# williamyang1991/FRESCO

Measured on AMD Instinct MI355X. Metric: denoising-steps/sec (8-frame batch, 512^2), FRESCO hot-path step, higher is better.
Workload: dtype f16; 1 GPU; cfg2 (BASELINE.json configs[1]): 8 frames 512x512, SD-1.5 decoder shapes, FRESCO attention only (3x up_blocks.2 HW=1024 C=640 + 3x up_blocks.3 HW=4096 C=320 processor calls per step, projections included), 15-step schedule 1x spatial+cf+temporal / 7x cf+temporal / 7x cf; parallelism=single GPU

## Files before the change

### fresco_amd/csrc/attn.hip

```cpp
#include "attn_cfg.h"
#include <type_traits>

namespace fresco {

template <int D>
__global__ __launch_bounds__(256) void kv_pack_kernel(const half_t* __restrict__ k,
                                                       const half_t* __restrict__ v,
                                                       const int32_t* __restrict__ kv_rows,
                                                       char* __restrict__ img, float* __restrict__ ktmax,
                                                       int H, int M, int nT, int64_t group_rows,
                                                       int64_t kv_ld) {
    using Cfg = AttnCfg<D>;
    const int tile = blockIdx.x, h = blockIdx.y, g = blockIdx.z;
    __shared__ int32_t rows[64];
    __shared__ __attribute__((aligned(16))) half_t ks[64][D + 8];
    __shared__ __attribute__((aligned(16))) half_t vs[64][D + 8];

    if (threadIdx.x < 64) {
        const int m = tile * 64 + threadIdx.x;
        int32_t r = -1;
        if (m < M) r = kv_rows ? kv_rows[m] : m;
        rows[threadIdx.x] = r;
    }
    __syncthreads();
// ... 30 lines not shown
        for (int e = 0; e < 8; ++e) {
            const int key = kc * 16 + (e & 3) + 8 * (e >> 2) + 4 * cc;
            half_t val = (half_t)0;
            if (d < D)
                val = vs[key][d];
            else if (Cfg::ONES && d == D && rows[key] >= 0)
                val = (half_t)1;
            o[e] = val;
        }
        *reinterpret_cast<half8_t*>(dst + Cfg::TILE + Cfg::KTILE + (int64_t)c * 16) = o;
    }
    {
        const int row = threadIdx.x >> 2, part = threadIdx.x & 3;
        float n2 = 0.f;
        for (int dc = part; dc < D / 8; dc += 4) {
            const half8_t kk = *reinterpret_cast<const half8_t*>(&ks[row][dc * 8]);
#pragma unroll
            for (int e = 0; e < 8; ++e) n2 = fmaf((float)kk[e], (float)kk[e], n2);
        }
        n2 += __shfl_xor(n2, 1, 64);
        n2 += __shfl_xor(n2, 2, 64);
#pragma unroll
        for (int off = 32; off >= 4; off >>= 1) n2 = fmaxf(n2, __shfl_xor(n2, off, 64));
        __shared__ float wmax[4];
        if ((threadIdx.x & 63) == 0) wmax[threadIdx.x >> 6] = n2;
        __syncthreads();
        if (threadIdx.x == 0)
            ktmax[(int64_t)(g * H + h) * nT + tile] = fmaxf(fmaxf(wmax[0], wmax[1]), fmaxf(wmax[2], wmax[3]));
    }
}

template <int KIN, int D>
struct KvProjCfg {
    static constexpr int ROWB = KIN * 2 + 16;
    static constexpr int HPW = 160 / D;
    static constexpr int NPART = D / 4;
    static constexpr int XS_BYTES = 64 * ROWB;
    static constexpr int LDS_BYTES = XS_BYTES + HPW * NPART * 64 * 4 + 64 * 4;
};

template <int KIN, int D>
__global__ __launch_bounds__(320, KIN == 320 ? 3 : 2) void kvproj_pack_kernel(const half_t* __restrict__ x, int64_t x_ld,
                                                           const int32_t* __restrict__ x_rows,
                                                           const half_t* __restrict__ Wk,
                                                           const half_t* __restrict__ Wv, char* __restrict__ img,
                                                           float* __restrict__ ktmax, int H, int M, int nT) {
    using Cfg = AttnCfg<D>;
    using PC = KvProjCfg<KIN, D>;
    constexpr int ROWB = PC::ROWB, HPW = PC::HPW, NPART = PC::NPART;
    constexpr int NKS = KIN / 16;
    constexpr int SK = 4;
    constexpr int NST = NKS / SK;
    constexpr int CPR = KIN / 8;
    constexpr int NXL = 64 * CPR / 320;
    static_assert(NKS % SK == 0 && (64 * CPR) % 320 == 0 && 160 % D == 0 && D % 8 == 0, "shapes");
    extern __shared__ __attribute__((aligned(16))) char smem[];
    char* xs = smem;
    float* n2p = reinterpret_cast<float*>(smem + PC::XS_BYTES);
    int32_t* rows = reinterpret_cast<int32_t*>(n2p + HPW * NPART * 64);
    const int tile = blockIdx.x, fg = blockIdx.y, g = blockIdx.z;
    const int tid = threadIdx.x, lane = tid & 63, wave = tid >> 6;
    const int l31 = lane & 31, hi = lane >> 5;

    if (tid < 64) {
        const int m = tile * 64 + tid;
        rows[tid] = m < M ? x_rows[(int64_t)g * M + m] : -1;
    }
    const int ft = fg * 5 + wave;
    const half_t* wkp = Wk + (int64_t)(ft * 32 + l31) * KIN + hi * 32;
    const half_t* wvp = Wv + (int64_t)(ft * 32 + l31) * KIN + hi * 32;
    half8_t fk[2][SK], fv[2][SK];
    auto fetch = [&](int st, int buf) __attribute__((always_inline)) {
#pragma unroll
        for (int i = 0; i < SK; ++i) {
            fk[buf][i] = *reinterpret_cast<const half8_t*>(wkp + st * 64 + i * 8);
            fv[buf][i] = *reinterpret_cast<const half8_t*>(wvp + st * 64 + i * 8);
        }
    };
    fetch(0, 0);
    __builtin_amdgcn_sched_barrier(0);
    __syncthreads();
    {
        uint4 xv[NXL];
#pragma unroll
        for (int i = 0; i < NXL; ++i) {
            const int c = tid + i * 320;
            const int row = c / CPR, dc = c % CPR;
            const int32_t r = rows[row];
            xv[i] = make_uint4(0, 0, 0, 0);
            if (r >= 0) xv[i] = *reinterpret_cast<const uint4*>(x + (int64_t)r * x_ld + dc * 8);
        }
        __builtin_amdgcn_sched_barrier(0);
#pragma unroll
        for (int i = 0; i < NXL; ++i) {
            const int c = tid + i * 320;
            *reinterpret_cast<uint4*>(xs + (c / CPR) * ROWB + (c % CPR) * 16) = xv[i];
        }
    }
    floatx16 ak[2], av[2];
#pragma unroll
    for (int b = 0; b < 2; ++b)
#pragma unroll
        for (int r = 0; r < 16; ++r) ak[b][r] = av[b][r] = 0.f;
    __syncthreads();
#pragma unroll
    for (int st = 0; st < NST; ++st) {
        const int buf = st & 1;
        if (st + 1 < NST) fetch(st + 1, buf ^ 1);
        __builtin_amdgcn_sched_barrier(0);
#pragma unroll
        for (int i = 0; i < SK; ++i) {
            const int kb = (st * 64 + hi * 32 + i * 8) * 2;
            const half8_t x0 = *reinterpret_cast<const half8_t*>(xs + l31 * ROWB + kb);
            const half8_t x1 = *reinterpret_cast<const half8_t*>(xs + (32 + l31) * ROWB + kb);
            ak[0] = __builtin_amdgcn_mfma_f32_32x32x16_f16(fk[buf][i], x0, ak[0], 0, 0, 0);
            ak[1] = __builtin_amdgcn_mfma_f32_32x32x16_f16(fk[buf][i], x1, ak[1], 0, 0, 0);
            av[0] = __builtin_amdgcn_mfma_f32_32x32x16_f16(x0, fv[buf][i], av[0], 0, 0, 0);
            av[1] = __builtin_amdgcn_mfma_f32_32x32x16_f16(x1, fv[buf][i], av[1], 0, 0, 0);
        }
        __builtin_amdgcn_sched_barrier(0);
    }
#pragma unroll
    for (int b = 0; b < 2; ++b) {
        const int key = b * 32 + l31;
#pragma unroll
        for (int j = 0; j < 4; ++j) {
            const int f0 = ft * 32 + 8 * j + 4 * hi;
            const int head = f0 / D, dd = f0 - head * D;
            half4_t w;
            float n2 = 0.f;
#pragma unroll
            for (int e = 0; e < 4; ++e) {
                w[e] = (half_t)ak[b][4 * j + e];
                n2 = fmaf((float)w[e], (float)w[e], n2);
            }
            char* dst = img + ((int64_t)(g * H + head) * (nT + 1) + tile) * Cfg::TILE;
            *reinterpret_cast<half4_t*>(dst + ((dd >> 3) * 64 + key) * 16 + (dd & 7) * 2) = w;
            n2p[((head - fg * HPW) * NPART + (dd >> 2)) * 64 + key] = n2;
        }
    }
    {
        const int f = ft * 32 + l31;
        const int head = f / D, d = f - head * D;
        char* dst = img + ((int64_t)(g * H + head) * (nT + 1) + tile + 1) * Cfg::TILE + Cfg::KTILE;
#pragma unroll
        for (int b = 0; b < 2; ++b)
#pragma unroll
            for (int kq = 0; kq < 2; ++kq) {
                half8_t w;
#pragma unroll
                for (int e = 0; e < 8; ++e) w[e] = (half_t)av[b][8 * kq + e];
                *reinterpret_cast<half8_t*>(dst + (((2 * b + kq) * 2 + hi) * Cfg::DPV + d) * 16) = w;
            }
    }
    {
        constexpr int KPAD = (Cfg::DPK - D) / 8;
        constexpr int VPAD = Cfg::DPV - D;
        constexpr int PER_HEAD = KPAD * 64 + VPAD * 8;
        for (int i = tid; i < HPW * PER_HEAD; i += 320) {
            const int hl = i / PER_HEAD, c = i % PER_HEAD;
            const int head = fg * HPW + hl;
            char* base = img + ((int64_t)(g * H + head) * (nT + 1) + tile) * Cfg::TILE;
            if (c < KPAD * 64) {
                const int pc = c / 64, key = c % 64;
                uint4 val = make_uint4(0, 0, 0, 0);
                if (Cfg::MCOL && pc == 0 && rows[key] >= 0) val.x = 0x3C00u;
                *reinterpret_cast<uint4*>(base + ((D / 8 + pc) * 64 + key) * 16) = val;
            } else {
                const int c2 = c - KPAD * 64;
                const int pr = c2 / 8, kcc = c2 % 8;
                const int kc = kcc >> 1, cc = kcc & 1;
                half8_t o;
#pragma unroll
                for (int e = 0; e < 8; ++e) {
                    const int key = kc * 16 + (e & 3) + 8 * (e >> 2) + 4 * cc;
                    o[e] = (Cfg::ONES && pr == 0 && rows[key] >= 0) ? (half_t)1 : (half_t)0;
                }
                *reinterpret_cast<half8_t*>(base + Cfg::TILE + Cfg::KTILE + (kcc * Cfg::DPV + D + pr) * 16) = o;
            }
        }
    }
    __syncthreads();
    if (wave < HPW) {
        float n2 = 0.f;
#pragma unroll
        for (int p_ = 0; p_ < NPART; ++p_) n2 += n2p[(wave * NPART + p_) * 64 + lane];
#pragma unroll
        for (int off = 32; off > 0; off >>= 1) n2 = fmaxf(n2, __shfl_xor(n2, off, 64));
        if (lane == 0) ktmax[(int64_t)(g * H + fg * HPW + wave) * nT + tile] = n2;
    }
}

template <int N>
__device__ __forceinline__ void ring_wait_barrier() {
    asm volatile("s_waitcnt vmcnt(%0) lgkmcnt(0)\n\ts_barrier" ::"n"(N) : "memory");
}

template <int D, int QB>
__global__ __launch_bounds__(512, 2) void attn_flash_kernel(const half_t* __restrict__ q,
                                                          const char* __restrict__ img,
                                                          const float* __restrict__ ktmax,
                                                          half_t* __restrict__ out, int B, int H, int Lq,
                                                          int M, int nT, int batch_per_group,
                                                          float scale_log2, float diag_bias_log2, int64_t q_ld) {
    using Cfg = AttnCfg<D>;
    extern __shared__ __attribute__((aligned(16))) char smem[];
    constexpr int ROWS = 256 * QB;

    const int nQblk = (Lq + ROWS - 1) / ROWS;
    const unsigned blk = blockIdx.x;
    const int h = blk % H;
    const int qblk = (blk / H) % nQblk;
    const int b = blk / (H * nQblk);
    const int g = b / batch_per_group;
    const int C = H * D;

    const int tid = threadIdx.x;
    const int lane = tid & 63, wave = tid >> 6;
    const int l31 = lane & 31, hi = lane >> 5;
    const int qrow0 = qblk * ROWS + wave * 32 * QB + l31;
    const int wave_s = __builtin_amdgcn_readfirstlane(wave);
    const int grpB = wave_s >= 4 ? 1 : 0;

    half8_t qf[QB][Cfg::NKS];
    float q2[QB];
#pragma unroll
    for (int j = 0; j < QB; ++j) {
        const int qr = qrow0 + 32 * j;
        const half_t* qp = q + ((int64_t)b * Lq + (qr < Lq ? qr : Lq - 1)) * q_ld + h * D;
        q2[j] = 0.f;
#pragma unroll
        for (int ks = 0; ks < Cfg::NKS; ++ks) {
            const int d0 = ks * 16 + hi * 8;
            half8_t t = {0, 0, 0, 0, 0, 0, 0, 0};
            if (d0 < D) t = *reinterpret_cast<const half8_t*>(qp + d0);
#pragma unroll
            for (int e = 0; e < 8; ++e) q2[j] = fmaf((float)t[e], (float)t[e], q2[j]);
            qf[j][ks] = t;
        }
        q2[j] += __shfl_xor(q2[j], 32, 64);
    }

    float kmax;
    {
        const float* km = ktmax + (int64_t)(g * H + h) * nT;
        float k2 = 0.f;
        for (int i = lane; i < nT; i += 64) k2 = fmaxf(k2, km[i]);
#pragma unroll
        for (int off = 32; off > 0; off >>= 1) k2 = fmaxf(k2, __shfl_xor(k2, off, 64));
        kmax = sqrtf(k2);
// ... 226 lines not shown
            for (int db = 0; db < Cfg::NDB; ++db)
#pragma unroll
                for (int j = 0; j < QB; ++j) {
                    o[j][db] = __builtin_amdgcn_mfma_f32_32x32x16_f16(vf[kc][db], pf[j][kc], o[j][db], 0, 0, 0);
                }
        __builtin_amdgcn_sched_barrier(0);
        if (!LAST) qk(kf);
        __builtin_amdgcn_s_setprio(0);
        __builtin_amdgcn_sched_barrier(0);
    };

    const std::integral_constant<bool, true> yes;
    const std::integral_constant<bool, false> no_last, no;
    const std::integral_constant<bool, true> fast;
    {
        int u = 0;
        if (nT > 1) {
            step(0, no_last, no);
            u = 1;
            if (!need_diag) {
                bool safe = true;
#pragma unroll
                for (int j = 0; j < QB; ++j) safe = safe && (cmul * (qbound[j] - m_run[j]) <= NOMAX_THR);
                nomax = __builtin_amdgcn_readfirstlane((int)__all(safe));
            }
            if (!need_diag)
                for (; u + 3 < nT; ++u) step(u, no_last, fast);
            for (; u < nT - 1; ++u) step(u, no_last, no);
        }
        nomax = 0;
        step(u, yes, no);
    }

#pragma unroll
    for (int j = 0; j < QB; ++j) {
        float l_tot;
        if (Cfg::ONES) {
            constexpr int rr = D % 32;
            l_tot = __shfl(o[j][D / 32][(rr & 3) + 4 * (rr >> 3)], l31 + 32 * ((rr >> 2) & 1), 64);
        } else {
            l_tot = l_run[j] + __shfl_xor(l_run[j], 32, 64);
        }
        const float inv = 1.f / l_tot;
        const int qr = qrow0 + 32 * j;
        {
            half_t* op = out + ((int64_t)b * Lq + (qr < Lq ? qr : 0)) * C + h * D;
#pragma unroll
            for (int db = 0; db < Cfg::NDB; ++db)
#pragma unroll
                for (int gp = 0; gp < 2; ++gp) {
                    const int dA = db * 32 + gp * 16;
                    if (dA >= D) continue;
                    half4_t wa, wb;
#pragma unroll
                    for (int jj = 0; jj < 4; ++jj) {
                        wa[jj] = (half_t)(o[j][db][(2 * gp) * 4 + jj] * inv);
                        wb[jj] = (half_t)(o[j][db][(2 * gp + 1) * 4 + jj] * inv);
                    }
                    if (dA + 8 < D) {
                        const u32x2 a = __builtin_bit_cast(u32x2, wa), bb = __builtin_bit_cast(u32x2, wb);
                        const auto s0 = __builtin_amdgcn_permlane32_swap(a[0], bb[0], false, false);
                        const auto s1 = __builtin_amdgcn_permlane32_swap(a[1], bb[1], false, false);
                        u32x4 st;
                        st[0] = s0[0]; st[1] = s1[0]; st[2] = s0[1]; st[3] = s1[1];
                        if (qr < Lq) *reinterpret_cast<u32x4*>(op + dA + hi * 8) = st;
                    } else if (qr < Lq) {
                        *reinterpret_cast<half4_t*>(op + dA + hi * 4) = wa;
                    }
                }
        }
    }
}

template <int D, int QB>
static int launch_flash(const half_t* q, const char* img, half_t* out, int B, int H, int Lq, int M, int nT,
                        int n_groups, float scale, float diag_bias, int64_t q_ld, const float* ktmax,
                        hipStream_t st) {
    using Cfg = AttnCfg<D>;
    if (int rc = allow_dyn_lds(&attn_flash_kernel<D, QB>, Cfg::LDS_BYTES)) return rc;
    const int nQblk = (Lq + 256 * QB - 1) / (256 * QB);
    const float log2e = 1.4426950408889634f;
    ProfScope ps(FRESCO_PROF_ATTN_FLASH, B * H, Lq, M, D, st);
    const int grid = H * nQblk * B;
    hipLaunchKernelGGL((attn_flash_kernel<D, QB>), dim3(grid), dim3(512), Cfg::LDS_BYTES, st, q, img,
                       ktmax, out, B, H, Lq, M, nT, B / n_groups, scale * log2e, diag_bias * log2e, q_ld);
    return check_launch();
}

template <int D>
static int launch_attn(const half_t* q, const half_t* k, const half_t* v, const int32_t* kv_rows,
                       half_t* out, char* ws, int B, int H, int Lq, int n_groups, int M,
                       int64_t group_rows, float scale, float diag_bias, int64_t q_ld, int64_t kv_ld,
                       hipStream_t st) {
    using Cfg = AttnCfg<D>;
    const int nT = ntiles_of(M);
    char* img = ws;
    float* ktmax = reinterpret_cast<float*>(ws + align_up((size_t)n_groups * H * (nT + 1) * Cfg::TILE, 256));
    dim3 pg(nT, H, n_groups);
    {
        ProfScope ps(FRESCO_PROF_KV_PACK, n_groups, H, M, D, st);
        hipLaunchKernelGGL((kv_pack_kernel<D>), pg, dim3(256), 0, st, k, v, kv_rows, img, ktmax, H, M, nT, group_rows,
                           kv_ld);
    }
    if constexpr (D <= 48 && Cfg::MCOL) {
        const int grid2 = H * ((Lq + 511) / 512) * B;
        if (Lq > 256 && grid2 < device_cus())
            return launch_flash<D, 1>(q, img, out, B, H, Lq, M, nT, n_groups, scale, diag_bias, q_ld, ktmax, st);
        return launch_flash<D, 2>(q, img, out, B, H, Lq, M, nT, n_groups, scale, diag_bias, q_ld, ktmax, st);
    } else {
        return launch_flash<D, 1>(q, img, out, B, H, Lq, M, nT, n_groups, scale, diag_bias, q_ld, ktmax, st);
    }
}

static size_t attn_ws_bytes(int n_groups, int H, int M, int D) {
    const size_t nT = ntiles_of(M);
    const size_t dpk = (D + 15) / 16 * 16, dpv = (D + 31) / 32 * 32;
    return align_up((size_t)n_groups * H * (nT + 1) * ((dpk + dpv) * 128), 256) +
           align_up((size_t)n_groups * H * nT * sizeof(float), 256);
}

}

using namespace fresco;

extern "C" size_t fresco_attn_workspace_bytes(int n_groups, int H, int M, int D) {
    if (n_groups <= 0 || H <= 0 || M <= 0 || D <= 0) return 0;
    return attn_ws_bytes(n_groups, H, M, D);
}

extern "C" int fresco_attn_fwd_ld(const void* q, const void* k, const void* v, const int32_t* kv_rows,
                                  void* out, void* workspace, size_t workspace_bytes, int B, int H,
                                  int Lq, int D, int n_groups, int M, int64_t group_rows, float scale,
                                  float diag_bias, int64_t q_ld, int64_t kv_ld, void* stream) {
    if (!q || !k || !v || !out || !workspace) return FRESCO_EINVAL;
    if (q_ld < (int64_t)H * D || kv_ld < (int64_t)H * D || q_ld % 8 != 0 || kv_ld % 8 != 0) return FRESCO_EINVAL;
    if (B <= 0 || H <= 0 || Lq <= 0 || D <= 0 || n_groups <= 0 || M <= 0 || group_rows <= 0)
        return FRESCO_EINVAL;
    if (B % n_groups != 0 || !(scale > 0.f)) return FRESCO_EINVAL;
    if (workspace_bytes < attn_ws_bytes(n_groups, H, M, D)) return FRESCO_EWORKSPACE;
    hipStream_t st = as_stream(stream);
    const half_t* qh = static_cast<const half_t*>(q);
    const half_t* kh = static_cast<const half_t*>(k);
    const half_t* vh = static_cast<const half_t*>(v);
    half_t* oh = static_cast<half_t*>(out);
    char* ws = static_cast<char*>(workspace);
#define FRESCO_ATTN_CASE(DD)                                                                       \
    case DD:                                                                                       \
        return launch_attn<DD>(qh, kh, vh, kv_rows, oh, ws, B, H, Lq, n_groups, M, group_rows, scale, \
                               diag_bias, q_ld, kv_ld, st);
    switch (D) {
        FRESCO_ATTN_CASE(8)
        FRESCO_ATTN_CASE(16)
        FRESCO_ATTN_CASE(32)
        FRESCO_ATTN_CASE(40)
        FRESCO_ATTN_CASE(64)
        FRESCO_ATTN_CASE(80)
        FRESCO_ATTN_CASE(96)
        FRESCO_ATTN_CASE(128)
        default:
            return FRESCO_EUNSUPPORTED;
    }
#undef FRESCO_ATTN_CASE
}

namespace fresco {
template <int KIN, int D>
static int launch_kvproj_attn(const half_t* q, const half_t* x, int64_t x_ld, const int32_t* x_rows, const half_t* Wk,
                              const half_t* Wv, half_t* out, char* ws, int B, int H, int Lq, int n_groups, int M,
                              float scale, int64_t q_ld, hipStream_t st) {
    using Cfg = AttnCfg<D>;
    const int nT = ntiles_of(M);
    char* img = ws;
    float* ktmax = reinterpret_cast<float*>(ws + align_up((size_t)n_groups * H * (nT + 1) * Cfg::TILE, 256));
    {
        ProfScope ps(FRESCO_PROF_KV_PACK, n_groups, H, M, -D, st);
        constexpr int lds = KvProjCfg<KIN, D>::LDS_BYTES;
        if (int rc = allow_dyn_lds(&kvproj_pack_kernel<KIN, D>, lds)) return rc;
        hipLaunchKernelGGL((kvproj_pack_kernel<KIN, D>), dim3(nT, H * D / 160, n_groups), dim3(320), lds, st, x, x_ld, x_rows,
                           Wk, Wv, img, ktmax, H, M, nT);
    }
    if constexpr (D <= 48 && Cfg::MCOL) {
        const int grid2 = H * ((Lq + 511) / 512) * B;
        if (Lq > 256 && grid2 < device_cus())
            return launch_flash<D, 1>(q, img, out, B, H, Lq, M, nT, n_groups, scale, 0.f, q_ld, ktmax, st);
        return launch_flash<D, 2>(q, img, out, B, H, Lq, M, nT, n_groups, scale, 0.f, q_ld, ktmax, st);
    } else {
        return launch_flash<D, 1>(q, img, out, B, H, Lq, M, nT, n_groups, scale, 0.f, q_ld, ktmax, st);
    }
}
}

extern "C" int fresco_attn_kvproj_supported(int H, int D, int K_in) {
    return (H > 0 && (int64_t)H * D == K_in && ((D == 40 && K_in == 320) || (D == 80 && K_in == 640))) ? 1 : 0;
}

extern "C" int fresco_attn_fwd_kvproj(const void* q, const void* x, int64_t x_ld, const int32_t* x_rows, const void* Wk,
                                      const void* Wv, void* out, void* workspace, size_t workspace_bytes, int B, int H,
                                      int Lq, int D, int n_groups, int M, int K_in, float scale, int64_t q_ld,
                                      void* stream) {
    if (!q || !x || !x_rows || !Wk || !Wv || !out || !workspace) return FRESCO_EINVAL;
    if (B <= 0 || H <= 0 || Lq <= 0 || D <= 0 || n_groups <= 0 || M <= 0 || K_in <= 0) return FRESCO_EINVAL;
    if (B % n_groups != 0 || !(scale > 0.f)) return FRESCO_EINVAL;
    if (q_ld < (int64_t)H * D || q_ld % 8 != 0 || x_ld < K_in || x_ld % 8 != 0) return FRESCO_EINVAL;
    if (!fresco_attn_kvproj_supported(H, D, K_in)) return FRESCO_EUNSUPPORTED;
    if (workspace_bytes < attn_ws_bytes(n_groups, H, M, D)) return FRESCO_EWORKSPACE;
    hipStream_t st = as_stream(stream);
    const half_t* qh = static_cast<const half_t*>(q);
    const half_t* xh = static_cast<const half_t*>(x);
    const half_t* wk = static_cast<const half_t*>(Wk);
    const half_t* wv = static_cast<const half_t*>(Wv);
    half_t* oh = static_cast<half_t*>(out);
    char* ws = static_cast<char*>(workspace);
    if (D == 40)
        return launch_kvproj_attn<320, 40>(qh, xh, x_ld, x_rows, wk, wv, oh, ws, B, H, Lq, n_groups, M, scale, q_ld, st);
    return launch_kvproj_attn<640, 80>(qh, xh, x_ld, x_rows, wk, wv, oh, ws, B, H, Lq, n_groups, M, scale, q_ld, st);
}

extern "C" int fresco_attn_fwd(const void* q, const void* k, const void* v, const int32_t* kv_rows,
                               void* out, void* workspace, size_t workspace_bytes, int B, int H,
                               int Lq, int D, int n_groups, int M, int64_t group_rows, float scale,
                               float diag_bias, void* stream) {
// ... 4 lines not shown
```

Measured before the change: 486.6 denoising-steps/sec.

## Stage KV-projection weights via LDS DMA ring and stage packed tiles in LDS

Rewrites the fused K/V projection-and-pack kernel so weights are streamed into a 3-slot swizzled LDS ring with global_load_lds DMA instead of per-lane register fetches. For the C=320 case each block now processes two 64-key tiles, which amortizes weight traffic. Output K/V tiles are assembled in LDS and written out with coalesced 16-byte copies, and key norms are recomputed from the staged tile. In exchange the kernel uses about 145KB of LDS, which likely caps occupancy at one block per CU despite the launch bounds, and it relies on inline asm with hand-managed waitcnt.

```diff
diff --git a/fresco_amd/csrc/attn.hip b/fresco_amd/csrc/attn.hip
--- a/fresco_amd/csrc/attn.hip
+++ b/fresco_amd/csrc/attn.hip
@@ -86,12 +86,27 @@
 
 template <int KIN, int D>
 struct KvProjCfg {
+    static constexpr int NKT = KIN == 320 ? 2 : 1;
+    static constexpr int NKEY = NKT * 64;
     static constexpr int ROWB = KIN * 2 + 16;
     static constexpr int HPW = 160 / D;
-    static constexpr int NPART = D / 4;
-    static constexpr int XS_BYTES = 64 * ROWB;
-    static constexpr int LDS_BYTES = XS_BYTES + HPW * NPART * 64 * 4 + 64 * 4;
+    static constexpr int KC = 64;
+    static constexpr int SLOT = 160 * KC * 2;
+    static constexpr int NSLOT = 3;
+    static constexpr int XS_BYTES = NKEY * ROWB;
+    static constexpr int RING_OFF = XS_BYTES;
+    static constexpr int ROWS_OFF = RING_OFF + NSLOT * SLOT;
+    static constexpr int LDS_BYTES = ROWS_OFF + NKEY * 4;
+    static constexpr int OUT_BYTES = HPW * NKT * AttnCfg<D>::TILE;
+    static_assert(OUT_BYTES <= ROWS_OFF && SLOT % (5 * 1024) == 0 && XS_BYTES % 16 == 0, "LDS plan");
 };
+
+static_assert(KvProjCfg<320, 40>::LDS_BYTES == 145920 && KvProjCfg<640, 80>::LDS_BYTES == 144640, "the header's LDS plan");
+
+template <int N>
+__device__ __forceinline__ void kvproj_wait_barrier() {
+    asm volatile("s_waitcnt vmcnt(%0) lgkmcnt(0)\n\ts_barrier" ::"n"(N) : "memory");
+}
 
 template <int KIN, int D>
 __global__ __launch_bounds__(320, KIN == 320 ? 3 : 2) void kvproj_pack_kernel(const half_t* __restrict__ x, int64_t x_ld,
@@ -101,38 +116,48 @@
                                                            float* __restrict__ ktmax, int H, int M, int nT) {
     using Cfg = AttnCfg<D>;
     using PC = KvProjCfg<KIN, D>;
-    constexpr int ROWB = PC::ROWB, HPW = PC::HPW, NPART = PC::NPART;
-    constexpr int NKS = KIN / 16;
-    constexpr int SK = 4;
-    constexpr int NST = NKS / SK;
+    constexpr int ROWB = PC::ROWB, HPW = PC::HPW, NKT = PC::NKT, NKEY = PC::NKEY;
+    constexpr int NC = KIN / PC::KC;
+    constexpr int NCH = 2 * NC;
+    constexpr int NT32 = 2 * NKT;
     constexpr int CPR = KIN / 8;
-    constexpr int NXL = 64 * CPR / 320;
-    static_assert(NKS % SK == 0 && (64 * CPR) % 320 == 0 && 160 % D == 0 && D % 8 == 0, "shapes");
+    constexpr int NXL = NKEY * CPR / 320;
+    constexpr int NPW = PC::SLOT / (5 * 1024);
+    static_assert(KIN % PC::KC == 0 && (NKEY * CPR) % 320 == 0 && 160 % D == 0 && D % 8 == 0, "shapes");
     extern __shared__ __attribute__((aligned(16))) char smem[];
     char* xs = smem;
-    float* n2p = reinterpret_cast<float*>(smem + PC::XS_BYTES);
-    int32_t* rows = reinterpret_cast<int32_t*>(n2p + HPW * NPART * 64);
-    const int tile = blockIdx.x, fg = blockIdx.y, g = blockIdx.z;
+    char* ring = smem + PC::RING_OFF;
+    int32_t* rows = reinterpret_cast<int32_t*>(smem + PC::ROWS_OFF);
+    const int tp = blockIdx.x, fg = blockIdx.y, g = blockIdx.z;
     const int tid = threadIdx.x, lane = tid & 63, wave = tid >> 6;
     const int l31 = lane & 31, hi = lane >> 5;
-
-    if (tid < 64) {
-        const int m = tile * 64 + tid;
+    const int wave_s = __builtin_amdgcn_readfirstlane(wave);
+
+    uint32_t dma_off[NPW];
+#pragma unroll
+    for (int i = 0; i < NPW; ++i) {
+        const int row = (i * 5 + wave_s) * 8 + (lane >> 3);
+        dma_off[i] = (uint32_t)(row * KIN * 2 + (((lane & 7) ^ ((row >> 1) & 7)) * 16));
+    }
+    const uint32_t lds0 =
+        __builtin_amdgcn_readfirstlane((uint32_t)(size_t)(__attribute__((address_space(3))) char*)smem);
+    auto stage = [&](int ch, int slot) __attribute__((always_inline)) {
+        const half_t* W = ch < NC ? Wk : Wv;
+        const char* src = reinterpret_cast<const char*>(W + (int64_t)fg * 160 * KIN + (ch % NC) * PC::KC);
+        const uint32_t dstb = lds0 + PC::RING_OFF + slot * PC::SLOT + wave_s * 1024;
+#pragma unroll
+        for (int i = 0; i < NPW; ++i) {
+            const uint32_t m0v = dstb + i * 5 * 1024;
+            asm volatile("s_mov_b32 m0, %2\n\tglobal_load_lds_dwordx4 %0, %1" ::"v"(dma_off[i]), "s"(src), "s"(m0v)
+                         : "memory");
+        }
+    };
+    stage(0, 0);
+    stage(1, 1);
+    if (tid < NKEY) {
+        const int m = tp * NKEY + tid;
         rows[tid] = m < M ? x_rows[(int64_t)g * M + m] : -1;
     }
-    const int ft = fg * 5 + wave;
-    const half_t* wkp = Wk + (int64_t)(ft * 32 + l31) * KIN + hi * 32;
-    const half_t* wvp = Wv + (int64_t)(ft * 32 + l31) * KIN + hi * 32;
-    half8_t fk[2][SK], fv[2][SK];
-    auto fetch = [&](int st, int buf) __attribute__((always_inline)) {
-#pragma unroll
-        for (int i = 0; i < SK; ++i) {
-            fk[buf][i] = *reinterpret_cast<const half8_t*>(wkp + st * 64 + i * 8);
-            fv[buf][i] = *reinterpret_cast<const half8_t*>(wvp + st * 64 + i * 8);
-        }
-    };
-    fetch(0, 0);
-    __builtin_amdgcn_sched_barrier(0);
     __syncthreads();
     {
         uint4 xv[NXL];
@@ -151,74 +176,96 @@
             *reinterpret_cast<uint4*>(xs + (c / CPR) * ROWB + (c % CPR) * 16) = xv[i];
         }
     }
-    floatx16 ak[2], av[2];
-#pragma unroll
-    for (int b = 0; b < 2; ++b)
-#pragma unroll
-        for (int r = 0; r < 16; ++r) ak[b][r] = av[b][r] = 0.f;
+    floatx16 acc[NT32];
+    half4_t kp[NT32][4];
+#pragma unroll
+    for (int t = 0; t < NT32; ++t)
+#pragma unroll
+        for (int r = 0; r < 16; ++r) acc[t][r] = 0.f;
+    kvproj_wait_barrier<0>();
+    const int wrow = wave * 32 + l31;
+    const char* wfrag = ring + wrow * 128;
+    const int wsw = (wrow >> 1) & 7;
+    const char* xfrag = xs + l31 * ROWB + hi * 16;
+#pragma unroll
+    for (int ch = 0; ch < NCH; ++ch) {
+        if (ch > 0) {
+            if (ch + 1 < NCH) kvproj_wait_barrier<NPW>(); else kvproj_wait_barrier<0>();
+        }
+        if (ch + 2 < NCH) stage(ch + 2, (ch + 2) % PC::NSLOT);
+        __builtin_amdgcn_sched_barrier(0);
+        const char* wsl = wfrag + (ch % PC::NSLOT) * PC::SLOT;
+        const int kc = ch % NC;
+#pragma unroll
+        for (int i = 0; i < PC::KC / 16; ++i) {
+            const half8_t fw = *reinterpret_cast<const half8_t*>(wsl + (((2 * i + hi) ^ wsw) * 16));
+            half8_t fx[NT32];
+#pragma unroll
+            for (int t = 0; t < NT32; ++t)
+                fx[t] = *reinterpret_cast<const half8_t*>(xfrag + t * 32 * ROWB + (kc * PC::KC + i * 16) * 2);
+#pragma unroll
+            for (int t = 0; t < NT32; ++t) {
+                if (ch < NC)
+                    acc[t] = __builtin_amdgcn_mfma_f32_32x32x16_f16(fw, fx[t], acc[t], 0, 0, 0);
+                else
+                    acc[t] = __builtin_amdgcn_mfma_f32_32x32x16_f16(fx[t], fw, acc[t], 0, 0, 0);
+            }
+        }
+        if (ch == NC - 1) {
+#pragma unroll
+            for (int t = 0; t < NT32; ++t)
+#pragma unroll
+                for (int j = 0; j < 4; ++j) {
+#pragma unroll
+                    for (int e = 0; e < 4; ++e) kp[t][j][e] = (half_t)acc[t][4 * j + e];
+                }
+#pragma unroll
+            for (int t = 0; t < NT32; ++t)
+#pragma unroll
+                for (int r = 0; r < 16; ++r) acc[t][r] = 0.f;
+        }
+    }
     __syncthreads();
-#pragma unroll
-    for (int st = 0; st < NST; ++st) {
-        const int buf = st & 1;
-        if (st + 1 < NST) fetch(st + 1, buf ^ 1);
-        __builtin_amdgcn_sched_barrier(0);
-#pragma unroll
-        for (int i = 0; i < SK; ++i) {
-            const int kb = (st * 64 + hi * 32 + i * 8) * 2;
-            const half8_t x0 = *reinterpret_cast<const half8_t*>(xs + l31 * ROWB + kb);
-            const half8_t x1 = *reinterpret_cast<const half8_t*>(xs + (32 + l31) * ROWB + kb);
-            ak[0] = __builtin_amdgcn_mfma_f32_32x32x16_f16(fk[buf][i], x0, ak[0], 0, 0, 0);
-            ak[1] = __builtin_amdgcn_mfma_f32_32x32x16_f16(fk[buf][i], x1, ak[1], 0, 0, 0);
-            av[0] = __builtin_amdgcn_mfma_f32_32x32x16_f16(x0, fv[buf][i], av[0], 0, 0, 0);
-            av[1] = __builtin_amdgcn_mfma_f32_32x32x16_f16(x1, fv[buf][i], av[1], 0, 0, 0);
-        }
-        __builtin_amdgcn_sched_barrier(0);
-    }
-#pragma unroll
-    for (int b = 0; b < 2; ++b) {
-        const int key = b * 32 + l31;
+    char* ob = smem;
+#pragma unroll
+    for (int t = 0; t < NT32; ++t) {
+        const int kt = t >> 1, key = (t & 1) * 32 + l31;
 #pragma unroll
         for (int j = 0; j < 4; ++j) {
-            const int f0 = ft * 32 + 8 * j + 4 * hi;
-            const int head = f0 / D, dd = f0 - head * D;
-            half4_t w;
-            float n2 = 0.f;
-#pragma unroll
-            for (int e = 0; e < 4; ++e) {
-                w[e] = (half_t)ak[b][4 * j + e];
-                n2 = fmaf((float)w[e], (float)w[e], n2);
-            }
-            char* dst = img + ((int64_t)(g * H + head) * (nT + 1) + tile) * Cfg::TILE;
-            *reinterpret_cast<half4_t*>(dst + ((dd >> 3) * 64 + key) * 16 + (dd & 7) * 2) = w;
-            n2p[((head - fg * HPW) * NPART + (dd >> 2)) * 64 + key] = n2;
-        }
-    }
-    {
-        const int f = ft * 32 + l31;
-        const int head = f / D, d = f - head * D;
-        char* dst = img + ((int64_t)(g * H + head) * (nT + 1) + tile + 1) * Cfg::TILE + Cfg::KTILE;
-#pragma unroll
-        for (int b = 0; b < 2; ++b)
+            const int f0 = wave * 32 + 8 * j + 4 * hi;
+            const int hl = f0 / D, dd = f0 - hl * D;
+            *reinterpret_cast<half4_t*>(ob + (hl * NKT + kt) * Cfg::TILE + ((dd >> 3) * 64 + key) * 16 + (dd & 7) * 2) =
+                kp[t][j];
+        }
+    }
+    {
+        const int fl = wave * 32 + l31;
+        const int hl = fl / D, d = fl - hl * D;
+#pragma unroll
+        for (int t = 0; t < NT32; ++t) {
+            const int kt = t >> 1, b = t & 1;
 #pragma unroll
             for (int kq = 0; kq < 2; ++kq) {
                 half8_t w;
 #pragma unroll
-                for (int e = 0; e < 8; ++e) w[e] = (half_t)av[b][8 * kq + e];
-                *reinterpret_cast<half8_t*>(dst + (((2 * b + kq) * 2 + hi) * Cfg::DPV + d) * 16) = w;
-            }
+                for (int e = 0; e < 8; ++e) w[e] = (half_t)acc[t][8 * kq + e];
+                *reinterpret_cast<half8_t*>(ob + (hl * NKT + kt) * Cfg::TILE + Cfg::KTILE +
+                                            (((2 * b + kq) * 2 + hi) * Cfg::DPV + d) * 16) = w;
+            }
+        }
     }
     {
         constexpr int KPAD = (Cfg::DPK - D) / 8;
         constexpr int VPAD = Cfg::DPV - D;
-        constexpr int PER_HEAD = KPAD * 64 + VPAD * 8;
-        for (int i = tid; i < HPW * PER_HEAD; i += 320) {
-            const int hl = i / PER_HEAD, c = i % PER_HEAD;
-            const int head = fg * HPW + hl;
-            char* base = img + ((int64_t)(g * H + head) * (nT + 1) + tile) * Cfg::TILE;
+        constexpr int PER_TILE = KPAD * 64 + VPAD * 8;
+        for (int i = tid; i < HPW * NKT * PER_TILE; i += 320) {
+            const int it = i / PER_TILE, c = i % PER_TILE;
+            const int32_t* rw = rows + (it % NKT) * 64;
+            char* base = ob + it * Cfg::TILE;
             if (c < KPAD * 64) {
                 const int pc = c / 64, key = c % 64;
                 uint4 val = make_uint4(0, 0, 0, 0);
-                if (Cfg::MCOL && pc == 0 && rows[key] >= 0) val.x = 0x3C00u;
+                if (Cfg::MCOL && pc == 0 && rw[key] >= 0) val.x = 0x3C00u;
                 *reinterpret_cast<uint4*>(base + ((D / 8 + pc) * 64 + key) * 16) = val;
             } else {
                 const int c2 = c - KPAD * 64;
@@ -228,20 +275,38 @@
 #pragma unroll
                 for (int e = 0; e < 8; ++e) {
                     const int key = kc * 16 + (e & 3) + 8 * (e >> 2) + 4 * cc;
-                    o[e] = (Cfg::ONES && pr == 0 && rows[key] >= 0) ? (half_t)1 : (half_t)0;
-                }
-                *reinterpret_cast<half8_t*>(base + Cfg::TILE + Cfg::KTILE + (kcc * Cfg::DPV + D + pr) * 16) = o;
+                    o[e] = (Cfg::ONES && pr == 0 && rw[key] >= 0) ? (half_t)1 : (half_t)0;
+                }
+                *reinterpret_cast<half8_t*>(base + Cfg::KTILE + (kcc * Cfg::DPV + D + pr) * 16) = o;
             }
         }
     }
     __syncthreads();
-    if (wave < HPW) {
+    {
+        constexpr int PPT = Cfg::TILE / 16, KP = Cfg::KTILE / 16;
+        constexpr int NPC = HPW * NKT * PPT;
+#pragma unroll 4
+        for (int i = tid; i < NPC; i += 320) {
+            const int it = i / PPT, p = i - it * PPT;
+            const int tile = tp * NKT + it % NKT, head = fg * HPW + it / NKT;
+            const uint4 v = *reinterpret_cast<const uint4*>(ob + i * 16);
+            if (tile < nT)
+                *reinterpret_cast<uint4*>(img + ((int64_t)(g * H + head) * (nT + 1) + tile + (p >= KP ? 1 : 0)) * Cfg::TILE +
+                                          p * 16) = v;
+        }
+    }
+    for (int it = wave_s; it < HPW * NKT; it += 5) {
+        const int tile = tp * NKT + it % NKT;
         float n2 = 0.f;
 #pragma unroll
-        for (int p_ = 0; p_ < NPART; ++p_) n2 += n2p[(wave * NPART + p_) * 64 + lane];
+        for (int dc = 0; dc < D / 8; ++dc) {
+            const half8_t kk = *reinterpret_cast<const half8_t*>(ob + it * Cfg::TILE + (dc * 64 + lane) * 16);
+#pragma unroll
+            for (int e = 0; e < 8; ++e) n2 = fmaf((float)kk[e], (float)kk[e], n2);
+        }
 #pragma unroll
         for (int off = 32; off > 0; off >>= 1) n2 = fmaxf(n2, __shfl_xor(n2, off, 64));
-        if (lane == 0) ktmax[(int64_t)(g * H + fg * HPW + wave) * nT + tile] = n2;
+        if (lane == 0 && tile < nT) ktmax[(int64_t)(g * H + fg * HPW + it / NKT) * nT + tile] = n2;
     }
 }
 
@@ -706,7 +771,8 @@
         ProfScope ps(FRESCO_PROF_KV_PACK, n_groups, H, M, -D, st);
         constexpr int lds = KvProjCfg<KIN, D>::LDS_BYTES;
         if (int rc = allow_dyn_lds(&kvproj_pack_kernel<KIN, D>, lds)) return rc;
-        hipLaunchKernelGGL((kvproj_pack_kernel<KIN, D>), dim3(nT, H * D / 160, n_groups), dim3(320), lds, st, x, x_ld, x_rows,
+        constexpr int NKT = KvProjCfg<KIN, D>::NKT;
+        hipLaunchKernelGGL((kvproj_pack_kernel<KIN, D>), dim3((nT + NKT - 1) / NKT, H * D / 160, n_groups), dim3(320), lds, st, x, x_ld, x_rows,
                            Wk, Wv, img, ktmax, H, M, nT);
     }
     if constexpr (D <= 48 && Cfg::MCOL) {
```

New measurement: 489.5 denoising-steps/sec, median of 6. Within noise of the previous version (+0.6%).

## Add QB=2 flash path for D=80 splitting key tiles into halves

Applied to the files above, without the earlier changes.

Adds a specialized flash-attention body for head dim 80 that processes 512 query rows per block (two 32-row groups per wave) and splits each 64-key tile into two 32-key half-phases. It uses a no-running-max fast path and interleaves PV and next QK MFMAs. A block-wide vote falls back to two QB=1 passes when the no-rescale bound cannot be guaranteed. The aim is to reuse each staged K/V tile across twice the query rows and raise MFMA density for the D=80 (up_blocks.2) calls. The cost is much higher register pressure and extra LDS for votes, with a launch heuristic now choosing QB=2 for D=80 unless the grid underfills the device.

```diff
diff --git a/fresco_amd/csrc/attn.hip b/fresco_amd/csrc/attn.hip
--- a/fresco_amd/csrc/attn.hip
+++ b/fresco_amd/csrc/attn.hip
@@ -251,25 +251,64 @@
 }
 
 template <int D, int QB>
-__global__ __launch_bounds__(512, 2) void attn_flash_kernel(const half_t* __restrict__ q,
-                                                          const char* __restrict__ img,
-                                                          const float* __restrict__ ktmax,
-                                                          half_t* __restrict__ out, int B, int H, int Lq,
-                                                          int M, int nT, int batch_per_group,
-                                                          float scale_log2, float diag_bias_log2, int64_t q_ld) {
+__device__ __forceinline__ void flash_store(const floatx16 (&o)[QB][AttnCfg<D>::NDB], const float (&l_run)[QB],
+                                            half_t* __restrict__ out, int64_t row0, int Lq, int C, int h, int qrow0,
+                                            int l31, int hi) {
+    using Cfg = AttnCfg<D>;
+#pragma unroll
+    for (int j = 0; j < QB; ++j) {
+        float l_tot;
+        if (Cfg::ONES) {
+            constexpr int rr = D % 32;
+            l_tot = __shfl(o[j][D / 32][(rr & 3) + 4 * (rr >> 3)], l31 + 32 * ((rr >> 2) & 1), 64);
+        } else {
+            l_tot = l_run[j] + __shfl_xor(l_run[j], 32, 64);
+        }
+        const float inv = 1.f / l_tot;
+        const int qr = qrow0 + 32 * j;
+        {
+            half_t* op = out + (row0 + (qr < Lq ? qr : 0)) * C + h * D;
+#pragma unroll
+            for (int db = 0; db < Cfg::NDB; ++db)
+#pragma unroll
+                for (int gp = 0; gp < 2; ++gp) {
+                    const int dA = db * 32 + gp * 16;
+                    if (dA >= D) continue;
+                    half4_t wa, wb;
+#pragma unroll
+                    for (int jj = 0; jj < 4; ++jj) {
+                        wa[jj] = (half_t)(o[j][db][(2 * gp) * 4 + jj] * inv);
+                        wb[jj] = (half_t)(o[j][db][(2 * gp + 1) * 4 + jj] * inv);
+                    }
+                    if (dA + 8 < D) {
+                        const u32x2 a = __builtin_bit_cast(u32x2, wa), bb = __builtin_bit_cast(u32x2, wb);
+                        const auto s0 = __builtin_amdgcn_permlane32_swap(a[0], bb[0], false, false);
+                        const auto s1 = __builtin_amdgcn_permlane32_swap(a[1], bb[1], false, false);
+                        u32x4 st;
+                        st[0] = s0[0]; st[1] = s1[0]; st[2] = s0[1]; st[3] = s1[1];
+                        if (qr < Lq) *reinterpret_cast<u32x4*>(op + dA + hi * 8) = st;
+                    } else if (qr < Lq) {
+                        *reinterpret_cast<half4_t*>(op + dA + hi * 4) = wa;
+                    }
+                }
+        }
+    }
+}
+
+template <int D, int QB>
+struct FlashHalves : std::integral_constant<bool, D == 80 && QB == 2> {};
+
+template <int D, int QB>
+__device__ __forceinline__ void flash_body(const half_t* __restrict__ q, const char* __restrict__ img,
+                                           const float* __restrict__ ktmax, half_t* __restrict__ out, int H, int Lq,
+                                           int M, int nT, int batch_per_group, float scale_log2,
+                                           float diag_bias_log2, int64_t q_ld, int h, int qblk, int b, int tid) {
     using Cfg = AttnCfg<D>;
     extern __shared__ __attribute__((aligned(16))) char smem[];
     constexpr int ROWS = 256 * QB;
-
-    const int nQblk = (Lq + ROWS - 1) / ROWS;
-    const unsigned blk = blockIdx.x;
-    const int h = blk % H;
-    const int qblk = (blk / H) % nQblk;
-    const int b = blk / (H * nQblk);
     const int g = b / batch_per_group;
     const int C = H * D;
 
-    const int tid = threadIdx.x;
     const int lane = tid & 63, wave = tid >> 6;
     const int l31 = lane & 31, hi = lane >> 5;
     const int qrow0 = qblk * ROWS + wave * 32 * QB + l31;
@@ -562,44 +601,368 @@
         step(u, yes, no);
     }
 
-#pragma unroll
-    for (int j = 0; j < QB; ++j) {
-        float l_tot;
-        if (Cfg::ONES) {
-            constexpr int rr = D % 32;
-            l_tot = __shfl(o[j][D / 32][(rr & 3) + 4 * (rr >> 3)], l31 + 32 * ((rr >> 2) & 1), 64);
+    flash_store<D, QB>(o, l_run, out, (int64_t)b * Lq, Lq, C, h, qrow0, l31, hi);
+}
+
+template <int X>
+__device__ __forceinline__ float lane_xor(float v) {
+    return __builtin_bit_cast(float, __builtin_amdgcn_ds_swizzle(__builtin_bit_cast(int, v), (X << 10) | 0x1f));
+}
+__device__ __forceinline__ void both_halves(float v, float& a, float& b) {
+    const unsigned u = __builtin_bit_cast(unsigned, v);
+    const auto sw = __builtin_amdgcn_permlane32_swap(u, u, false, false);
+    a = __builtin_bit_cast(float, (unsigned)sw[0]);
+    b = __builtin_bit_cast(float, (unsigned)sw[1]);
+}
+
+template <int D>
+__device__ __forceinline__ void flash_body_halves(const half_t* __restrict__ q, const char* __restrict__ img,
+                                                  const float* __restrict__ ktmax, half_t* __restrict__ out, int H,
+                                                  int Lq, int M, int nT, int batch_per_group, float scale_log2,
+                                                  float diag_bias_log2, int64_t q_ld, int h, int qblk, int b) {
+    using Cfg = AttnCfg<D>;
+    static_assert(!Cfg::MCOL && Cfg::ONES, "head dims with a spare V^T row and no spare K column (D = 80)");
+    constexpr int NKS = Cfg::NKS, NDB = Cfg::NDB;
+    extern __shared__ __attribute__((aligned(16))) char smem[];
+    const int g = b / batch_per_group;
+    const int C = H * D;
+
+    const int tid = threadIdx.x;
+    const int lane = tid & 63, wave = tid >> 6;
+    const int l31 = lane & 31, hi = lane >> 5;
+    const int qrow0 = qblk * 512 + wave * 64 + l31;
+    const int wave_s = __builtin_amdgcn_readfirstlane(wave);
+    const int grpB = wave_s >= 4 ? 1 : 0;
+
+    half8_t qf[2][NKS];
+    float q2[2];
+#pragma unroll
+    for (int j = 0; j < 2; ++j) {
+        const int qr = qrow0 + 32 * j;
+        const half_t* qp = q + ((int64_t)b * Lq + (qr < Lq ? qr : Lq - 1)) * q_ld + h * D;
+        q2[j] = 0.f;
+#pragma unroll
+        for (int ks = 0; ks < NKS; ++ks) {
+            const half8_t t = *reinterpret_cast<const half8_t*>(qp + ks * 16 + hi * 8);
+#pragma unroll
+            for (int e = 0; e < 8; ++e) q2[j] = fmaf((float)t[e], (float)t[e], q2[j]);
+#pragma unroll
+            for (int e = 0; e < 8; ++e) qf[j][ks][e] = (half_t)((float)t[e] * scale_log2);
+        }
+        float qa, qb;
+        both_halves(q2[j], qa, qb);
+        q2[j] = qa + qb;
+    }
+    float kmax;
+    {
+        const float* km = ktmax + (int64_t)(g * H + h) * nT;
+        float k2 = 0.f;
+        for (int i = lane; i < nT; i += 64) k2 = fmaxf(k2, km[i]);
+        k2 = fmaxf(k2, lane_xor<16>(k2));
+        k2 = fmaxf(k2, lane_xor<8>(k2));
+        k2 = fmaxf(k2, lane_xor<4>(k2));
+        k2 = fmaxf(k2, lane_xor<2>(k2));
+        k2 = fmaxf(k2, lane_xor<1>(k2));
+        float ka, kb;
+        both_halves(k2, ka, kb);
+        kmax = sqrtf(fmaxf(ka, kb));
+    }
+    bool common = diag_bias_log2 == 0.f && nT >= 2;
+#pragma unroll
+    for (int j = 0; j < 2; ++j) common = common && (scale_log2 * sqrtf(q2[j]) * kmax <= FOLD_MAX);
+
+    constexpr int NPW_LO = Cfg::NP / 8, NPW_HI = (Cfg::NP + 7) / 8, NREM = Cfg::NP % 8;
+    const int many = wave_s < NREM ? 1 : 0;
+    const uint32_t lds0 =
+        __builtin_amdgcn_readfirstlane((uint32_t)(size_t)(__attribute__((address_space(3))) char*)smem);
+    const char* src = img + (int64_t)(g * H + h) * (nT + 1) * Cfg::TILE;
+    const uint32_t lane_off = (wave * 64 + lane) * 16;
+    auto stage = [&](int p, int slot) __attribute__((always_inline)) {
+        const char* sp = src + (int64_t)p * Cfg::TILE;
+        const uint32_t dstb = lds0 + slot * Cfg::TILE + wave_s * 1024;
+#pragma unroll
+        for (int i = 0; i < NPW_HI; ++i) {
+            if (i < NPW_LO || many) {
+                const uint32_t m0v = dstb + i * 8192;
+                asm volatile("s_mov_b32 m0, %2\n\tglobal_load_lds_dwordx4 %0, %1" ::"v"(lane_off), "s"(sp), "s"(m0v)
+                             : "memory");
+                sp += 8192;
+            }
+        }
+    };
+    auto wait_barrier = [&](int keep) __attribute__((always_inline)) {
+        if (keep == 0) {
+            ring_wait_barrier<0>();
+        } else if (many) {
+            if (keep == 1) ring_wait_barrier<NPW_HI>(); else ring_wait_barrier<2 * NPW_HI>();
         } else {
-            l_tot = l_run[j] + __shfl_xor(l_run[j], 32, 64);
-        }
-        const float inv = 1.f / l_tot;
-        const int qr = qrow0 + 32 * j;
+            if (keep == 1) ring_wait_barrier<NPW_LO>(); else ring_wait_barrier<2 * NPW_LO>();
+        }
+    };
+
+    const int koff = (hi * 64 + l31) * 16;
+    const int voff = Cfg::KTILE + (hi * Cfg::DPV + l31) * 16;
+    floatx16 s[2];
+    auto qk_half = [&](floatx16 (&acc)[2], int slot, int f, float c0, float c1) __attribute__((always_inline)) {
+        half8_t kf[NKS];
+        const char* kb_ = smem + slot * Cfg::TILE + koff + f * 512;
+#pragma unroll
+        for (int ks = 0; ks < NKS; ++ks) kf[ks] = *reinterpret_cast<const half8_t*>(kb_ + ks * 2048);
+#pragma unroll
+        for (int r = 0; r < 16; ++r) {
+            acc[0][r] = c0;
+            acc[1][r] = c1;
+        }
+#pragma unroll
+        for (int ks = 0; ks < NKS; ++ks)
+#pragma unroll
+            for (int j = 0; j < 2; ++j)
+                acc[j] = __builtin_amdgcn_mfma_f32_32x32x16_f16(kf[ks], qf[j][ks], acc[j], 0, 0, 0);
+    };
+
+    stage(0, 3);
+    stage(1, 0);
+    if (nT > 1) stage(2, 1);
+    if (nT > 2) stage(3, 2);
+    wait_barrier(nT > 2 ? 2 : (nT > 1 ? 1 : 0));
+    float m_run[2];
+    {
+        floatx16 t[2];
+        qk_half(t, 3, 1, 0.f, 0.f);
+        qk_half(s, 3, 0, 0.f, 0.f);
+#pragma unroll
+        for (int j = 0; j < 2; ++j) {
+            float mt = fmaxf(s[j][0], t[j][0]);
+#pragma unroll
+            for (int r = 1; r < 16; ++r) mt = fmaxf(fmaxf(mt, s[j][r]), t[j][r]);
+            const unsigned mb = __builtin_bit_cast(unsigned, mt);
+            const auto sw = __builtin_amdgcn_permlane32_swap(mb, mb, false, false);
+            m_run[j] = fmaxf(__builtin_bit_cast(float, (unsigned)sw[0]), __builtin_bit_cast(float, (unsigned)sw[1]));
+            common = common && (scale_log2 * sqrtf(q2[j]) * kmax * 1.001f + 1e-3f - m_run[j] <= NOMAX_THR);
+        }
+    }
+    __builtin_amdgcn_sched_barrier(0);
+
+    {
+        int* votes = reinterpret_cast<int*>(smem + Cfg::LDS_BYTES);
+        const int mine = __builtin_amdgcn_readfirstlane((int)__all(common));
+        if (lane == 0) votes[wave] = mine;
+        __syncthreads();
+        int all = 1;
+#pragma unroll
+        for (int w = 0; w < 8; ++w) all &= votes[w];
+        if (__builtin_amdgcn_readfirstlane(all) == 0) {
+#pragma nounroll
+            for (int half = 0; half < 2; ++half) {
+                ring_wait_barrier<0>();
+                int tid_ = tid, h_ = h, qb_ = qblk * 2 + half, b_ = b;
+                asm volatile("" : "+v"(tid_), "+s"(h_), "+s"(qb_), "+s"(b_));
+                if (qb_ * 256 < Lq)
+                    flash_body<D, 1>(q, img, ktmax, out, H, Lq, M, nT, batch_per_group, scale_log2, diag_bias_log2, q_ld,
+                                     h_, qb_, b_, tid_);
+            }
+            return;
+        }
+    }
+
+    floatx16 o[2][NDB];
+#pragma unroll
+    for (int j = 0; j < 2; ++j)
+#pragma unroll
+        for (int db = 0; db < NDB; ++db)
+#pragma unroll
+            for (int r = 0; r < 16; ++r) o[j][db][r] = 0.f;
+
+    auto phase = [&](int u, auto f_c, auto first_c, auto full_c) __attribute__((always_inline)) {
+        constexpr int F = decltype(f_c)::value;
+        constexpr bool FIRST = decltype(first_c)::value;
+        constexpr bool FULL = decltype(full_c)::value;
+        const int slot = u & 3;
+        auto ring_sync = [&]() __attribute__((always_inline)) {
+            if (F == 0) {
+                if (FULL) ring_wait_barrier<NPW_LO>(); else wait_barrier(u + 2 < nT ? 1 : 0);
+            } else {
+                asm volatile("s_waitcnt lgkmcnt(0)\n\ts_barrier" ::: "memory");
+                if (FULL || u + 3 < nT) stage(u + 4, (u + 3) & 3);
+            }
+        };
+        if (grpB) ring_sync();
+        __builtin_amdgcn_sched_barrier(0);
+
+        half8_t vf[2][NDB];
         {
-            half_t* op = out + ((int64_t)b * Lq + (qr < Lq ? qr : 0)) * C + h * D;
-#pragma unroll
-            for (int db = 0; db < Cfg::NDB; ++db)
-#pragma unroll
-                for (int gp = 0; gp < 2; ++gp) {
-                    const int dA = db * 32 + gp * 16;
-                    if (dA >= D) continue;
-                    half4_t wa, wb;
-#pragma unroll
-                    for (int jj = 0; jj < 4; ++jj) {
-                        wa[jj] = (half_t)(o[j][db][(2 * gp) * 4 + jj] * inv);
-                        wb[jj] = (half_t)(o[j][db][(2 * gp + 1) * 4 + jj] * inv);
-                    }
-                    if (dA + 8 < D) {
-                        const u32x2 a = __builtin_bit_cast(u32x2, wa), bb = __builtin_bit_cast(u32x2, wb);
-                        const auto s0 = __builtin_amdgcn_permlane32_swap(a[0], bb[0], false, false);
-                        const auto s1 = __builtin_amdgcn_permlane32_swap(a[1], bb[1], false, false);
-                        u32x4 st;
-                        st[0] = s0[0]; st[1] = s1[0]; st[2] = s0[1]; st[3] = s1[1];
-                        if (qr < Lq) *reinterpret_cast<u32x4*>(op + dA + hi * 8) = st;
-                    } else if (qr < Lq) {
-                        *reinterpret_cast<half4_t*>(op + dA + hi * 4) = wa;
-                    }
+            const char* vb_ = smem + slot * Cfg::TILE + voff + F * (4 * Cfg::DPV * 16);
+#pragma unroll
+            for (int kc = 0; kc < 2; ++kc)
+#pragma unroll
+                for (int db = 0; db < NDB; ++db)
+                    vf[kc][db] = *reinterpret_cast<const half8_t*>(vb_ + (kc * 2 * Cfg::DPV + db * 32) * 16);
+        }
+        __builtin_amdgcn_sched_barrier(0);
+
+        half8_t pf[2][2];
+#pragma unroll
+        for (int j = 0; j < 2; ++j) {
+            if (FIRST) {
+#pragma unroll
+                for (int r = 0; r < 16; ++r) s[j][r] -= m_run[j];
+            }
+#pragma unroll
+            for (int r = 0; r < 16; r += 2) {
+                const float p0 = __builtin_amdgcn_exp2f(s[j][r]);
+                const float p1 = __builtin_amdgcn_exp2f(s[j][r + 1]);
+                pf[j][r >> 3][r & 7] = (half_t)p0;
+                pf[j][r >> 3][(r & 7) + 1] = (half_t)p1;
+            }
+#pragma unroll
+            for (int kc = 0; kc < 2; ++kc) asm volatile("" : "+v"(pf[j][kc]));
+        }
+        __builtin_amdgcn_sched_barrier(0);
+
+        if (!grpB) ring_sync();
+        __builtin_amdgcn_sched_barrier(0);
+
+        half8_t kf[NKS];
+        {
+            const char* kb_ = smem + (F == 0 ? ((u + 3) & 3) * Cfg::TILE + 512 : slot * Cfg::TILE) + koff;
+#pragma unroll
+            for (int ks = 0; ks < NKS; ++ks) kf[ks] = *reinterpret_cast<const half8_t*>(kb_ + ks * 2048);
+        }
+        __builtin_amdgcn_sched_barrier(0);
+
+        __builtin_amdgcn_s_setprio(1);
+#pragma unroll
+        for (int kc = 0; kc < 2; ++kc)
+#pragma unroll
+            for (int db = 0; db < NDB; ++db)
+#pragma unroll
+                for (int j = 0; j < 2; ++j)
+                    o[j][db] = __builtin_amdgcn_mfma_f32_32x32x16_f16(vf[kc][db], pf[j][kc], o[j][db], 0, 0, 0);
+        __builtin_amdgcn_sched_barrier(0);
+#pragma unroll
+        for (int j = 0; j < 2; ++j)
+#pragma unroll
+            for (int r = 0; r < 16; ++r) s[j][r] = (FIRST && F == 0) ? 0.f : -m_run[j];
+#pragma unroll
+        for (int ks = 0; ks < NKS; ++ks)
+#pragma unroll
+            for (int j = 0; j < 2; ++j)
+                s[j] = __builtin_amdgcn_mfma_f32_32x32x16_f16(kf[ks], qf[j][ks], s[j], 0, 0, 0);
+        __builtin_amdgcn_s_setprio(0);
+        __builtin_amdgcn_sched_barrier(0);
+    };
+
+    const std::integral_constant<int, 0> f0;
+    const std::integral_constant<int, 1> f1;
+    const std::integral_constant<bool, true> yes;
+    const std::integral_constant<bool, false> no;
+    phase(0, f0, yes, no);
+    phase(0, f1, yes, no);
+    int u = 1;
+    for (; u + 3 < nT; ++u) {
+        phase(u, f0, no, yes);
+        phase(u, f1, no, yes);
+    }
+    for (; u < nT - 1; ++u) {
+        phase(u, f0, no, no);
+        phase(u, f1, no, no);
+    }
+
+    int tid2 = threadIdx.x;
+    asm volatile("" : "+v"(tid2));
+    const int l31e = tid2 & 31, hie = (tid2 >> 5) & 1;
+    {
+        const int slot = u & 3;
+        if (grpB) ring_wait_barrier<0>();
+        __builtin_amdgcn_sched_barrier(0);
+        floatx16 s1[2];
+        qk_half(s1, (u + 3) & 3, 1, -m_run[0], -m_run[1]);
+        __builtin_amdgcn_sched_barrier(0);
+        half8_t pf[2][4];
+#pragma unroll
+        for (int j = 0; j < 2; ++j) {
+            int kbase = u * 64 + 4 * hie;
+            asm volatile("" : "+v"(kbase));
+#pragma unroll
+            for (int r = 0; r < 16; ++r) {
+                const int key0 = kbase + (r & 3) + 8 * (r >> 2);
+                if (key0 >= M) s[j][r] = -1e30f;
+                if (key0 + 32 >= M) s1[j][r] = -1e30f;
+            }
+            float mt = fmaxf(s[j][0], s1[j][0]);
+#pragma unroll
+            for (int r = 1; r < 16; ++r) mt = fmaxf(fmaxf(mt, s[j][r]), s1[j][r]);
+            {
+                const unsigned mb = __builtin_bit_cast(unsigned, mt);
+                const auto sw = __builtin_amdgcn_permlane32_swap(mb, mb, false, false);
+                mt = fmaxf(__builtin_bit_cast(float, (unsigned)sw[0]), __builtin_bit_cast(float, (unsigned)sw[1]));
+            }
+            if (__builtin_amdgcn_readfirstlane((int)__any(mt > RESCALE_THR)) != 0) {
+                const float delta = fmaxf(mt, 0.f);
+                const float alpha = __builtin_amdgcn_exp2f(-delta);
+#pragma unroll
+                for (int r = 0; r < 16; ++r) {
+                    s[j][r] -= delta;
+                    s1[j][r] -= delta;
                 }
-        }
-    }
+#pragma unroll
+                for (int db = 0; db < NDB; ++db)
+#pragma unroll
+                    for (int r = 0; r < 16; ++r) o[j][db][r] *= alpha;
+            }
+#pragma unroll
+            for (int r = 0; r < 16; r += 2) {
+                const float p0 = __builtin_amdgcn_exp2f(s[j][r]);
+                const float p1 = __builtin_amdgcn_exp2f(s[j][r + 1]);
+                const float p2 = __builtin_amdgcn_exp2f(s1[j][r]);
+                const float p3 = __builtin_amdgcn_exp2f(s1[j][r + 1]);
+                pf[j][r >> 3][r & 7] = (half_t)p0;
+                pf[j][r >> 3][(r & 7) + 1] = (half_t)p1;
+                pf[j][2 + (r >> 3)][r & 7] = (half_t)p2;
+                pf[j][2 + (r >> 3)][(r & 7) + 1] = (half_t)p3;
+            }
+#pragma unroll
+            for (int kc = 0; kc < 4; ++kc) asm volatile("" : "+v"(pf[j][kc]));
+        }
+        __builtin_amdgcn_sched_barrier(0);
+        if (!grpB) ring_wait_barrier<0>();
+        __builtin_amdgcn_sched_barrier(0);
+        const char* vb_ = smem + slot * Cfg::TILE + voff;
+#pragma unroll
+        for (int kc = 0; kc < 4; ++kc) {
+            half8_t vf[NDB];
+#pragma unroll
+            for (int db = 0; db < NDB; ++db)
+                vf[db] = *reinterpret_cast<const half8_t*>(vb_ + (kc * 2 * Cfg::DPV + db * 32) * 16);
+#pragma unroll
+            for (int db = 0; db < NDB; ++db)
+#pragma unroll
+                for (int j = 0; j < 2; ++j)
+                    o[j][db] = __builtin_amdgcn_mfma_f32_32x32x16_f16(vf[db], pf[j][kc], o[j][db], 0, 0, 0);
+        }
+    }
+
+    const float no_l[2] = {0.f, 0.f};
+    flash_store<D, 2>(o, no_l, out, (int64_t)b * Lq, Lq, C, h, qblk * 512 + (tid2 >> 6) * 64 + l31e, l31e, hie);
+}
+
+template <int D, int QB>
+__global__ __launch_bounds__(512, 2) void attn_flash_kernel(const half_t* __restrict__ q,
+                                                          const char* __restrict__ img,
+                                                          const float* __restrict__ ktmax,
+                                                          half_t* __restrict__ out, int B, int H, int Lq,
+                                                          int M, int nT, int batch_per_group,
+                                                          float scale_log2, float diag_bias_log2, int64_t q_ld) {
+    const int nQblk = (Lq + 256 * QB - 1) / (256 * QB);
+    const unsigned blk = blockIdx.x;
+    const int h = blk % H;
+    const int qblk = (blk / H) % nQblk;
+    const int b = blk / (H * nQblk);
+    if constexpr (FlashHalves<D, QB>::value)
+        flash_body_halves<D>(q, img, ktmax, out, H, Lq, M, nT, batch_per_group, scale_log2, diag_bias_log2, q_ld, h, qblk, b);
+    else
+        flash_body<D, QB>(q, img, ktmax, out, H, Lq, M, nT, batch_per_group, scale_log2, diag_bias_log2, q_ld, h, qblk, b,
+                          threadIdx.x);
 }
 
 template <int D, int QB>
@@ -607,14 +970,31 @@
                         int n_groups, float scale, float diag_bias, int64_t q_ld, const float* ktmax,
                         hipStream_t st) {
     using Cfg = AttnCfg<D>;
-    if (int rc = allow_dyn_lds(&attn_flash_kernel<D, QB>, Cfg::LDS_BYTES)) return rc;
+    constexpr int lds = Cfg::LDS_BYTES + (FlashHalves<D, QB>::value ? 64 : 0);
+    if (int rc = allow_dyn_lds(&attn_flash_kernel<D, QB>, lds)) return rc;
     const int nQblk = (Lq + 256 * QB - 1) / (256 * QB);
     const float log2e = 1.4426950408889634f;
     ProfScope ps(FRESCO_PROF_ATTN_FLASH, B * H, Lq, M, D, st);
     const int grid = H * nQblk * B;
-    hipLaunchKernelGGL((attn_flash_kernel<D, QB>), dim3(grid), dim3(512), Cfg::LDS_BYTES, st, q, img,
+    hipLaunchKernelGGL((attn_flash_kernel<D, QB>), dim3(grid), dim3(512), lds, st, q, img,
                        ktmax, out, B, H, Lq, M, nT, B / n_groups, scale * log2e, diag_bias * log2e, q_ld);
     return check_launch();
+}
+
+template <int D>
+static int launch_flash_auto(const half_t* q, const char* img, half_t* out, int B, int H, int Lq, int M, int nT,
+                             int n_groups, float scale, float diag_bias, int64_t q_ld, const float* ktmax,
+                             hipStream_t st) {
+    using Cfg = AttnCfg<D>;
+    if constexpr ((D <= 48 && Cfg::MCOL) || FlashHalves<D, 2>::value) {
+        const int grid2 = H * ((Lq + 511) / 512) * B;
+        const bool idle = grid2 < device_cus();
+        if (FlashHalves<D, 2>::value ? (idle || Lq <= 256) : (idle && Lq > 256))
+            return launch_flash<D, 1>(q, img, out, B, H, Lq, M, nT, n_groups, scale, diag_bias, q_ld, ktmax, st);
+        return launch_flash<D, 2>(q, img, out, B, H, Lq, M, nT, n_groups, scale, diag_bias, q_ld, ktmax, st);
+    } else {
+        return launch_flash<D, 1>(q, img, out, B, H, Lq, M, nT, n_groups, scale, diag_bias, q_ld, ktmax, st);
+    }
 }
 
 template <int D>
@@ -632,14 +1012,7 @@
         hipLaunchKernelGGL((kv_pack_kernel<D>), pg, dim3(256), 0, st, k, v, kv_rows, img, ktmax, H, M, nT, group_rows,
                            kv_ld);
     }
-    if constexpr (D <= 48 && Cfg::MCOL) {
-        const int grid2 = H * ((Lq + 511) / 512) * B;
-        if (Lq > 256 && grid2 < device_cus())
-            return launch_flash<D, 1>(q, img, out, B, H, Lq, M, nT, n_groups, scale, diag_bias, q_ld, ktmax, st);
-        return launch_flash<D, 2>(q, img, out, B, H, Lq, M, nT, n_groups, scale, diag_bias, q_ld, ktmax, st);
-    } else {
-        return launch_flash<D, 1>(q, img, out, B, H, Lq, M, nT, n_groups, scale, diag_bias, q_ld, ktmax, st);
-    }
+    return launch_flash_auto<D>(q, img, out, B, H, Lq, M, nT, n_groups, scale, diag_bias, q_ld, ktmax, st);
 }
 
 static size_t attn_ws_bytes(int n_groups, int H, int M, int D) {
@@ -709,14 +1082,7 @@
         hipLaunchKernelGGL((kvproj_pack_kernel<KIN, D>), dim3(nT, H * D / 160, n_groups), dim3(320), lds, st, x, x_ld, x_rows,
                            Wk, Wv, img, ktmax, H, M, nT);
     }
-    if constexpr (D <= 48 && Cfg::MCOL) {
-        const int grid2 = H * ((Lq + 511) / 512) * B;
-        if (Lq > 256 && grid2 < device_cus())
-            return launch_flash<D, 1>(q, img, out, B, H, Lq, M, nT, n_groups, scale, 0.f, q_ld, ktmax, st);
-        return launch_flash<D, 2>(q, img, out, B, H, Lq, M, nT, n_groups, scale, 0.f, q_ld, ktmax, st);
-    } else {
-        return launch_flash<D, 1>(q, img, out, B, H, Lq, M, nT, n_groups, scale, 0.f, q_ld, ktmax, st);
-    }
+    return launch_flash_auto<D>(q, img, out, B, H, Lq, M, nT, n_groups, scale, 0.f, q_ld, ktmax, st);
 }
 }
 
```

Result: faster. 491.8 denoising-steps/sec before, 497.1 denoising-steps/sec after (median of 6 runs) (+1.1%).
